# rvp-group/srrg2_proslam

Measured on AMD Instinct MI355X. Metric: tracked frames/sec on KITTI-00 stereo (1241x376, ~2k kp); SE(3) vs ref, higher is better.
Workload: dtype u64 popcount (Hamming) + f32 (projection, Jacobians, 6x6 normal equations)

## Files before the change

### srrg2_proslam_amd/csrc/align.hip

```cpp
#include "prs_device.h"
#include "prs_host.h"
#include "prs_se3.h"

#include <math.h>
#include <string.h>

#include <type_traits>
#include <vector>

namespace prs {

constexpr int kAlignThreads = 256;
constexpr int kTerms        = 29;
constexpr uint32_t kNoneU32 = 0xffffffffu;
constexpr float kFltMax     = 3.402823466e+38f;

typedef unsigned int au32x4 __attribute__((ext_vector_type(4)));

struct AlignShared {
  float X[16];
  float A[16];
  float Sinv[16];
  float T[16];
  float Tprev[16];
// ... 1495 lines not shown
      const float dn2 = ((((dx6[0] * dx6[0] + dx6[1] * dx6[1]) + dx6[2] * dx6[2]) + dx6[3] * dx6[3]) + dx6[4] * dx6[4]) + dx6[5] * dx6[5];
      const bool small_step = g.a.step_norm_exit > 0.0f && step_ok && dn2 < g.a.step_norm_exit * g.a.step_norm_exit;
      uint32_t changed_bits = 0;
#pragma unroll
      for (int i = 0; i < 16; ++i) {
        changed_bits |= __float_as_uint(X[i]) ^ __float_as_uint(sh.X[i]);
        sh.X[i] = X[i];
      }
      float a16[16];
      pose_to_camera(g.a, sh.Sinv, X, a16);
#pragma unroll
      for (int i = 0; i < 16; ++i) {
        sh.A[i] = a16[i];
      }
      sh.decision = ((g.a.stop_at_fixed_point && changed_bits == 0u && (sh.converged || inlier_run)) || (small_step && (sh.converged || inlier_run))) ? 1 : 0;
    }
    __syncthreads();
    ALIGN_ACC(acc_solve);
    if (sh.decision) {
      if (!inlier_run && inlier_run_length(g.a) > 0) {
        it_align = g.a.max_iterations - 1;
        continue;
      }
      ++it_align;
      break;
    }
  }

  __syncthreads();
  if (g.mode == PRS_MODE_ALIGN && !split_search && g.a.keep_only_inlier_correspondences && sh.have_cls && !sh.error) {
    const int nc = sh.n_corr;
    int base     = 0;
    for (int c0 = 0; c0 < nc; c0 += T) {
      const int c     = c0 + tid;
      const bool keep = c < nc && clsbuf[c] == 0;
      prs_corr cr;
      if (keep) {
        cr = gcorr[c];
      }
      const unsigned long long bal = __ballot(keep);
      if (lane == 0) {
        sh.wave_tot[wave] = __popcll(bal);
      }
      __syncthreads();
      int pos = base + __popcll(bal & ((1ull << lane) - 1ull));
      for (int w = 0; w < T / 64; ++w) {
        pos += w < wave ? sh.wave_tot[w] : 0;
        base += sh.wave_tot[w];
      }
      if (keep) {
        gcorr[pos] = cr;
      }
      __syncthreads();
    }
    if (tid == 0) {
      sh.n_corr = base;
    }
    __syncthreads();
  }

  __syncthreads();
  if (tid < 16) {
    if (!split_search) {
      g.b.X[(size_t) frame * 16 + tid] = sh.X[tid];
    }
    gstate->local_map_in_sensor[tid]          = sh.T[tid];
    gstate->local_map_in_sensor_previous[tid] = sh.Tprev[tid];
  }
  for (int i = tid; i < 36; i += T) {
    gres->H[i] = sh.H[i];
  }
  if (tid < 6) {
    gres->b[tid] = sh.b[tid];
  }
  if (tid == 0) {
    gstate->search_radius_pixels = sh.radius;
    gstate->current_iteration    = sh.it;
    gstate->descriptor_distance  = sh.dd;
    gstate->database_leaf_range  = sh.kd_range;
    gstate->has_converged        = sh.converged;
    gstate->config_changed       = sh.config_changed;
    gstate->num_recomputes       = sh.num_recomputes;
    gstate->reserved             = (gstate->reserved & ~1) | sh.no_prune;
    g.b.n_corr[frame]            = sh.n_corr;
    gres->chi_inliers            = sh.chi_in;
    gres->chi_total              = sh.chi_tot;
    gres->mean_disparity         = sh.mean_disp;
    gres->num_inliers            = sh.n_inl;
    gres->num_outliers           = sh.n_out;
    gres->num_invalid            = sh.n_inv;
    gres->num_correspondences    = sh.n_corr;
    gres->status                 = sh.n_inl >= g.a.min_num_inliers ? 1 : 0;
    gres->iterations             = g.mode == PRS_MODE_ALIGN ? (ran_inlier_phase ? max_it : g.a.max_iterations) : 1;
    gres->iterations_executed    = executed;
    gres->warnings               = sh.error ? sh.error : sh.flags;
    if (split_search) {
      ctl->flags |= sh.flags;
      ctl->need_search = 0;
      gres->warnings   = sh.error ? sh.error : ctl->flags;
    }
    if (g.stamps) {
      unsigned long long* st = g.stamps + (size_t) frame * 16;
      st[0] = 0;
      for (int i = 0; i < 9; ++i) {
        st[i + 1] = st[i] + sh.stamp_acc[i];
      }
    }
  }
}

constexpr int kGnThreads = 128;
constexpr int kGnSlots   = 8;

struct GnShared {
  float X[16], T[16], Tprev[16];
  float H[36], b[6];
  float chi_in, chi_tot;
  float fcnt[3];
  float pad0;
  float A[16];
  float Sinv[16];
  float wsum[32];
  unsigned long long it;
  int converged, need_search, n_inl, n_out, n_inv, stop, flags;
  int pose_ok;
  int wave_tot[4];
};
static_assert(offsetof(GnShared, b) == offsetof(GnShared, H) + 36 * sizeof(float) && offsetof(GnShared, chi_in) == offsetof(GnShared, b) + 6 * sizeof(float) &&
                offsetof(GnShared, chi_tot) == offsetof(GnShared, chi_in) + sizeof(float) && offsetof(GnShared, fcnt) == offsetof(GnShared, chi_tot) + sizeof(float),
              "the summed slots are written through GnShared::H");

__device__ __forceinline__ bool gn_advance(const prs_aligner_params& a, const int extra, int& it_align, bool fixed_point, const int n_inl) {
  const bool was_inlier_run = it_align >= a.max_iterations;
  ++it_align;
  if (fixed_point && !was_inlier_run && extra > 0) {
    it_align    = a.max_iterations;
    fixed_point = false;
  }
  if (fixed_point) {
    return true;
  }
  if (it_align == a.max_iterations && extra > 0) {
    return n_inl < a.min_num_inliers;
  }
  return it_align >= a.max_iterations + extra;
}

template <bool SHIPPED_FORMS = false, int PLAIN = 0>
__device__ __forceinline__ void gn_solve_wave(const AlignArgs& g, GnShared& sh, const int frame, const int nc, const int stid, const bool inlier_run) {
  const int lane = stid;
  if (sh.pose_ok) {
    const int rrow = lane < 6 ? lane : 5;
    const int blk  = rrow >= 3 ? 1 : 0;
    const int ci   = rrow - 3 * blk;
    const float* Yb = &sh.H[18 * blk];
    const float Ri0 = sh.A[ci], Ri1 = sh.A[4 + ci], Ri2 = sh.A[8 + ci];
    float o[6];
#pragma unroll
    for (int cb = 0; cb < 2; ++cb) {
      float v[3];
#pragma unroll
      for (int c = 0; c < 3; ++c) {
        v[c] = fmaf(Ri2, Yb[12 + 3 * cb + c], fmaf(Ri1, Yb[6 + 3 * cb + c], Ri0 * Yb[3 * cb + c]));
      }
#pragma unroll
      for (int j = 0; j < 3; ++j) {
        o[3 * cb + j] = fmaf(v[2], sh.A[8 + j], fmaf(v[1], sh.A[4 + j], v[0] * sh.A[j]));
      }
    }
    const float bb = fmaf(Ri2, sh.b[3 * blk + 2], fmaf(Ri1, sh.b[3 * blk + 1], Ri0 * sh.b[3 * blk]));
    __builtin_amdgcn_fence(__ATOMIC_RELEASE, "wavefront");
    __builtin_amdgcn_wave_barrier();
    __builtin_amdgcn_fence(__ATOMIC_ACQUIRE, "wavefront");
    if (lane < 6) {
      float2* hw = reinterpret_cast<float2*>(&sh.H[6 * rrow]);
      hw[0]      = make_float2(o[0], o[1]);
      hw[1]      = make_float2(o[2], o[3]);
      hw[2]      = make_float2(o[4], o[5]);
      sh.b[rrow] = bb;
    }
    __builtin_amdgcn_fence(__ATOMIC_RELEASE, "wavefront");
    __builtin_amdgcn_wave_barrier();
    __builtin_amdgcn_fence(__ATOMIC_ACQUIRE, "wavefront");
  }
  if (stid == 0) {
    const int cc = (int) sh.fcnt[0];
    sh.n_inl     = cc & ((int) kClsOutUnit - 1);
    sh.n_out     = cc / (int) kClsOutUnit;
    sh.n_inv     = nc - sh.n_inl - sh.n_out;
  }
  {
    const int prow  = lane < 3 ? lane : 2;
    const float4 xr = *reinterpret_cast<const float4*>(&sh.X[4 * prow]);
    float H[36], b[6];
#pragma unroll
    for (int i = 0; i < 36; ++i) {
      H[i] = sh.H[i];
    }
#pragma unroll
    for (int i = 0; i < 6; ++i) {
      b[i] = sh.b[i];
    }
    if (PLAIN == 0 && g.b.prior) {
      const float* pr = g.b.prior + (size_t) frame * 42;
#pragma unroll
      for (int i = 0; i < 36; ++i) {
        H[i] += pr[i];
      }
#pragma unroll
      for (int i = 0; i < 6; ++i) {
        b[i] += pr[36 + i];
      }
    }
    if (PLAIN == 2 || (PLAIN == 0 && g.a.enable_motion_prior)) {
      float X[16];
#pragma unroll
      for (int i = 0; i < 16; ++i) {
        X[i] = sh.X[i];
      }
      add_motion_prior(g.a, g.prior_mean ? g.prior_mean + (size_t) frame * 16 : nullptr, X, H, b);
    }
    auto bcast = [](const float v, const int l) -> float { return __int_as_float(__builtin_amdgcn_readlane(__float_as_int(v), l)); };
    float dx[6];
    const bool ok = ldlt_solve6(H, b, g.a.damping, dx, !SHIPPED_FORMS && g.a.damping_form == PRS_DAMPING_IDENTITY);
    bool small_step = false;
    if (g.a.step_norm_exit > 0.0f) {
      const float n2 = ((((dx[0] * dx[0] + dx[1] * dx[1]) + dx[2] * dx[2]) + dx[3] * dx[3]) + dx[4] * dx[4]) + dx[5] * dx[5];
      small_step     = ok && n2 < g.a.step_norm_exit * g.a.step_norm_exit;
    }
    float D[16];
    tnq2t(dx, D);
    float4 xn;
    xn.x = (xr.x * D[0] + xr.y * D[4]) + xr.z * D[8];
    xn.y = (xr.x * D[1] + xr.y * D[5]) + xr.z * D[9];
    xn.z = (xr.x * D[2] + xr.y * D[6]) + xr.z * D[10];
    xn.w = ((xr.x * D[3] + xr.y * D[7]) + xr.z * D[11]) + xr.w;
    xn.x = ok ? xn.x : xr.x;
    xn.y = ok ? xn.y : xr.y;
    xn.z = ok ? xn.z : xr.z;
    xn.w = ok ? xn.w : xr.w;
    const uint32_t changed = (__float_as_uint(xn.x) ^ __float_as_uint(xr.x)) | (__float_as_uint(xn.y) ^ __float_as_uint(xr.y)) |
                             (__float_as_uint(xn.z) ^ __float_as_uint(xr.z)) | (__float_as_uint(xn.w) ^ __float_as_uint(xr.w));
    const bool any_changed = (__ballot(changed != 0u) & 7ull) != 0ull;
    float4 an = xn;
    if (PLAIN == 0 && g.a.with_sensor) {
      const float4 sr = *reinterpret_cast<const float4*>(&sh.Sinv[4 * prow]);
      const float4 x0 = {bcast(xn.x, 0), bcast(xn.y, 0), bcast(xn.z, 0), bcast(xn.w, 0)};
      const float4 x1 = {bcast(xn.x, 1), bcast(xn.y, 1), bcast(xn.z, 1), bcast(xn.w, 1)};
      const float4 x2 = {bcast(xn.x, 2), bcast(xn.y, 2), bcast(xn.z, 2), bcast(xn.w, 2)};
      an.x = (sr.x * x0.x + sr.y * x1.x) + sr.z * x2.x;
      an.y = (sr.x * x0.y + sr.y * x1.y) + sr.z * x2.y;
      an.z = (sr.x * x0.z + sr.y * x1.z) + sr.z * x2.z;
      an.w = ((sr.x * x0.w + sr.y * x1.w) + sr.z * x2.w) + sr.w;
    }
    const float rs = (an.x + an.y) + (an.z + an.w);
    const float fs = (bcast(rs, 0) + bcast(rs, 1)) + bcast(rs, 2);
    if (lane < 3) {
      *reinterpret_cast<float4*>(&sh.X[4 * lane]) = xn;
      *reinterpret_cast<float4*>(&sh.A[4 * lane]) = an;
    }
    if (stid == 0) {
      sh.stop    = ((g.a.stop_at_fixed_point && !any_changed && (sh.converged || inlier_run)) || (small_step && (sh.converged || inlier_run))) ? 1 : 0;
      sh.pose_ok = (fs - fs) == 0.0f ? 1 : 0;
    }
  }
}

__device__ __forceinline__ void gn_finder_bookkeeping(const AlignArgs& g, GnShared& sh, const int stid, const int nc, const int it_align, const int extra,
                                                      const bool fixed_point) {
    int next        = it_align;
    const bool over = gn_advance(g.a, extra, next, fixed_point, sh.n_inl);
    if (!over && next < g.a.max_iterations) {
      if (stid < 16) {
        sh.T[stid] = sh.A[stid];
      }
      if (!sh.converged) {
        const unsigned long long k  = g.f.number_of_solver_iterations_per_projection;
        const unsigned long long it = sh.it;
        if (k == 0 || it % k == 0 || it == 1) {
          if (stid == 0) {
            sh.need_search = 1;
          }
        } else {
          if (stid < 16) {
            sh.Tprev[stid] = sh.A[stid];
          }
          if (stid == 0) {
            sh.it = it + 1;
            if (nc == 0) {
              sh.flags |= PRS_WARN_NO_MATCHES;
            }
          }
        }
      } else if (stid == 0 && nc == 0) {
        sh.flags |= PRS_WARN_NO_MATCHES;
      }
    }
}

constexpr int kGnLdsSlots = 4;
constexpr size_t gn_lds_bytes(const int lds_slots) {
  return ((sizeof(GnShared) + 15) / 16) * 16 + (size_t) (lds_slots * 128 + 64) * 2 * sizeof(float4);
}
template <int SLOTS, int DIM, bool KEEP_CLS, int LDS_SLOTS = kGnLdsSlots, int WAVES = 4, int PLAIN = 0>
__global__ __launch_bounds__(128, WAVES) void gn_kernel(const AlignArgs g) {
  constexpr int THREADS = 128;
  constexpr int kGnLdsSlots = LDS_SLOTS;
  constexpr int kGnLdsRows  = LDS_SLOTS * 128 + 64;
  extern __shared__ __attribute__((aligned(16))) unsigned char smem[];
  const int tid   = threadIdx.x;
  const int lane  = tid & 63;
  const int wave  = tid >> 6;
  const int frame = blockIdx.x;
  const int solver = frame & 1;
  const int stid   = tid - 64 * solver;
  FrameCtl* ctl    = g.ctl + frame;
  constexpr int LS_IDX = (SLOTS < LDS_SLOTS ? SLOTS : LDS_SLOTS) + 1;
  const size_t fbase                    = (size_t) frame * (size_t) g.b.fixed_stride;
  const prs_corr* __restrict__ gcorr_in = g.b.corr + fbase;
  int fi[LS_IDX], mi[LS_IDX];
#pragma unroll
  for (int k = 0; k < LS_IDX; ++k) {
    const int c  = k * 128 + tid;
    const int cc = c < g.b.fixed_stride ? c : 0;
    fi[k]        = gcorr_in[cc].fixed_idx;
    mi[k]        = gcorr_in[cc].moving_idx;
  }
  if (ctl->done || ctl->need_search) {
    return;
  }
  GnShared& sh             = *reinterpret_cast<GnShared*>(smem);
  prs_pcf_state* gstate    = g.b.state + frame;
  prs_align_result* gres   = g.b.result + frame;
  const float4* gops       = g.ops + (size_t) frame * (size_t) g.max_fixed * 2;
  const int nc             = g.b.n_corr[frame];
  const float mean_dsp     = gres->mean_disparity;

  if (tid < 16) {
    sh.X[tid]     = g.b.X[(size_t) frame * 16 + tid];
    sh.T[tid]     = gstate->local_map_in_sensor[tid];
    sh.Tprev[tid] = gstate->local_map_in_sensor_previous[tid];
  }
  if (tid == 0) {
    sh.it          = gstate->current_iteration;
    sh.converged   = gstate->has_converged;
    sh.need_search = 0;
    sh.flags       = 0;
    sh.n_inl       = ctl->n_inl;
    sh.n_out       = ctl->n_out;
    sh.n_inv       = ctl->n_inv;
    sh.chi_in      = gres->chi_inliers;
    sh.chi_tot     = gres->chi_total;
    sh.stop        = 0;
    const float* gx = g.b.X + (size_t) frame * 16;
    float x[16], a16[16], si[16];
#pragma unroll
    for (int i = 0; i < 16; ++i) {
      x[i] = gx[i];
    }
    se3_inverse(g.a.sensor_in_robot, si);
    pose_to_camera(g.a, si, x, a16);
#pragma unroll
    for (int i = 0; i < 16; ++i) {
      sh.Sinv[i] = si[i];
      sh.A[i]    = a16[i];
    }
    const PoseRegs x0 = {a16[0], a16[1], a16[2], a16[3], a16[4], a16[5], a16[6], a16[7], a16[8], a16[9], a16[10], a16[11]};
    sh.pose_ok        = pose_is_finite(x0) ? 1 : 0;
  }
  for (int i = tid; i < 36; i += THREADS) {
    sh.H[i] = gres->H[i];
  }
  if (tid < 6) {
    sh.b[tid] = gres->b[tid];
  }
  constexpr int LS = SLOTS < kGnLdsSlots ? SLOTS : kGnLdsSlots;
  float4* lz = reinterpret_cast<float4*>(smem + ((sizeof(GnShared) + 15) / 16) * 16);
  constexpr int LROWS = SLOTS <= kGnLdsSlots ? SLOTS * THREADS : kGnLdsRows;
  float4* lp = lz + LROWS;
  const float4* __restrict__ gfix = reinterpret_cast<const float4*>(g.b.fixed) + fbase;
  const float4* __restrict__ gmov = reinterpret_cast<const float4*>(g.b.moving) + (size_t) frame * (size_t) g.b.moving_stride;
  if (nc > 0) {
    static_assert(LS_IDX == LS + 1, "index pairs of the parked rows");
    float4 zr[LS + 1], pr[LS + 1];
#pragma unroll
    for (int k = 0; k < LS + 1; ++k) {
      const bool live = k * THREADS + tid < nc;
      zr[k]           = gfix[live ? fi[k] : 0];
      pr[k]           = gmov[live ? mi[k] : 0];
    }
#pragma unroll
    for (int k = 0; k < LS + 1; ++k) {
      const int c = k * THREADS + tid;
      if (k * THREADS < nc && c < LROWS) {
        float4 z = c < nc ? zr[k] : make_float4(0.f, 0.f, 0.f, 0.f);
        z.w      = parked_translation_weight(g.a, z, mean_dsp, DIM != 0 ? 0 : g.a.translation_weight_form);
        lz[c]    = z;
        lp[c]    = c < nc ? pr[k] : make_float4(0.f, 0.f, 1.f, 1.f);
      }
    }
  }
  if (SLOTS > kGnLdsSlots) {
    float4* wops = g.ops + (size_t) frame * (size_t) g.max_fixed * 2;
#pragma unroll
    for (int k = LS; k < SLOTS; ++k) {
      const int c = k * THREADS + tid;
      if (c >= LROWS && c < nc) {
        const int fi    = gcorr_in[c].fixed_idx, mi = gcorr_in[c].moving_idx;
        float4 z        = gfix[fi];
        z.w             = parked_translation_weight(g.a, z, mean_dsp, DIM != 0 ? 0 : g.a.translation_weight_form);
        wops[2 * c]     = z;
        wops[2 * c + 1] = gmov[mi];
      }
    }
  }
  const int my_slot = (lane >> 1) & 31;
  const int sum_dst = gn_slot_destination(my_slot, (lane & 1) != 0);
  __syncthreads();

  int it_align = ctl->it_align;
  int executed = ctl->executed;
  bool done    = false;
  const int extra = PLAIN != 0 ? 0 : inlier_run_length(g.a);
  uint32_t cls_bits = 0;
  bool have_cls     = false;


  while (true) {
    ++executed;
    if (nc < g.a.min_num_correspondences) {
      if (tid == 0) {
        sh.n_inl = sh.n_out = sh.n_inv = 0;
        sh.chi_in = sh.chi_tot = 0.0f;
        sh.stop = (g.a.stop_at_fixed_point && (sh.converged || it_align >= g.a.max_iterations)) ? 1 : 0;
      }
      for (int i = tid; i < 36; i += THREADS) {
        sh.H[i] = 0.0f;
      }
      if (tid < 6) {
        sh.b[tid] = 0.0f;
      }
      have_cls = false;
      __syncthreads();
      if (wave == solver) {
        gn_finder_bookkeeping(g, sh, stid, nc, it_align, extra, sh.stop != 0);
      }
      __syncthreads();
    } else {
      const bool inlier_run = PLAIN == 0 && it_align >= g.a.max_iterations;
      have_cls              = true;
      cls_bits              = 0;
      const PoseRegs pose = {sh.A[0], sh.A[1], sh.A[2], sh.A[3], sh.A[4], sh.A[5], sh.A[6], sh.A[7], sh.A[8], sh.A[9], sh.A[10], sh.A[11]};
      const bool pose_ok  = __builtin_amdgcn_readfirstlane(sh.pose_ok) != 0;
      f2 acc[kPairs];
#pragma unroll
      for (int i = 0; i < kPairs; ++i) {
        acc[i] = f2{0.0f, 0.0f};
      }
      float code = 0.0f;
      if (pose_ok) {
#pragma unroll
        for (int k = 0; k < SLOTS; ++k) {
          const int c0 = k * THREADS;
          if (k == 0 || c0 + 64 * wave < nc) {
            const int c = c0 + tid;
            float4 z, p;
            if (k < LS || (k == LS && c0 + 64 * wave < LROWS)) {
              z = lz[c];
              p = lp[c];
            } else {
              const int cs = cold_copy(c);
              z   = c < nc ? gops[2 * cs] : make_float4(0.f, 0.f, 0.f, 1.f);
              p   = c < nc ? gops[2 * cs + 1] : make_float4(0.f, 0.f, 1.f, 1.f);
            }
            int cls;
            factor_accumulate<DIM, true>(g.a, pose, z, p, mean_dsp, c < nc, acc, code, cls, inlier_run);
            if (KEEP_CLS) {
              cls_bits |= (uint32_t) (cls & 3) << (2 * k);
            }
          }
        }
      } else if (KEEP_CLS) {
#pragma unroll
        for (int k = 0; k < SLOTS; ++k) {
          if (k * THREADS + tid < nc) {
            cls_bits |= 2u << (2 * k);
          }
        }
      }
      acc[kSlotCls >> 1].x = code;
      float tot = wave_sum_slots(acc, lane);
      if (wave != solver) {
        sh.wsum[my_slot] = tot;
      }
      __syncthreads();
      if (wave == solver) {
        tot = tot + sh.wsum[my_slot];
        tot = tot + 0.0f;
        (&sh.H[0])[sum_dst] = tot;
        __builtin_amdgcn_fence(__ATOMIC_RELEASE, "wavefront");
        __builtin_amdgcn_wave_barrier();
        __builtin_amdgcn_fence(__ATOMIC_ACQUIRE, "wavefront");
        gn_solve_wave<DIM != 0, PLAIN>(g, sh, frame, nc, stid, inlier_run);
        __builtin_amdgcn_fence(__ATOMIC_RELEASE, "wavefront");
        __builtin_amdgcn_wave_barrier();
        __builtin_amdgcn_fence(__ATOMIC_ACQUIRE, "wavefront");
        gn_finder_bookkeeping(g, sh, stid, nc, it_align, extra, sh.stop != 0);
      }
      __syncthreads();
    }
    if (gn_advance(g.a, extra, it_align, sh.stop != 0, sh.n_inl)) {
      done = true;
      break;
    }
    if (it_align < g.a.max_iterations && sh.need_search) {
      break;
    }
  }

  int nc_out = nc;
  __syncthreads();
  if (KEEP_CLS && done && g.a.keep_only_inlier_correspondences && have_cls) {
    prs_corr* __restrict__ gcorr = g.b.corr + (size_t) frame * (size_t) g.b.fixed_stride;
    int base                     = 0;
#pragma unroll
    for (int k = 0; k < SLOTS; ++k) {
      const int c0 = k * THREADS;
      if (c0 < nc) {
        const int c     = c0 + tid;
        const bool keep = c < nc && ((cls_bits >> (2 * k)) & 3u) == 0u;
        prs_corr cr;
        if (keep) {
          cr = gcorr[c];
        }
        const unsigned long long bal = __ballot(keep);
        if (lane == 0) {
          sh.wave_tot[wave] = __popcll(bal);
        }
        __syncthreads();
        int pos = base + __popcll(bal & ((1ull << lane) - 1ull));
#pragma unroll
        for (int w = 0; w < THREADS / 64; ++w) {
          pos += w < wave ? sh.wave_tot[w] : 0;
          base += sh.wave_tot[w];
        }
        if (keep) {
          gcorr[pos] = cr;
        }
        __syncthreads();
      }
    }
    nc_out = base;
  }

  __syncthreads();
  if (tid < 16) {
    g.b.X[(size_t) frame * 16 + tid]           = sh.X[tid];
    gstate->local_map_in_sensor[tid]          = sh.T[tid];
    gstate->local_map_in_sensor_previous[tid] = sh.Tprev[tid];
  }
  for (int i = tid; i < 36; i += THREADS) {
    const int r = i / 6, c = i - 6 * r;
    gres->H[i]  = sh.H[r >= c ? i : 6 * c + r];
  }
  if (tid < 6) {
    gres->b[tid] = sh.b[tid];
  }
  if (tid == 0) {
    gstate->current_iteration = sh.it;
    gres->chi_inliers         = sh.chi_in;
    gres->chi_total           = sh.chi_tot;
    gres->num_inliers         = sh.n_inl;
    gres->num_outliers        = sh.n_out;
    gres->num_invalid         = sh.n_inv;
    gres->num_correspondences = nc_out;
    if (nc_out != nc) {
      g.b.n_corr[frame] = nc_out;
    }
    gres->status              = sh.n_inl >= g.a.min_num_inliers ? 1 : 0;
    gres->iterations          = it_align > g.a.max_iterations ? g.a.max_iterations + extra : g.a.max_iterations;
    gres->iterations_executed = executed;
    ctl->flags |= sh.flags;
    gres->warnings   = ctl->flags;
    ctl->it_align    = it_align;
    ctl->executed    = executed;
    ctl->n_inl       = sh.n_inl;
    ctl->n_out       = sh.n_out;
    ctl->n_inv       = sh.n_inv;
    ctl->need_search = done ? 0 : 1;
    ctl->done        = done ? 1 : 0;
    if (!done) {
      atomicAdd(g.pending, 1);
    }
  }
}

__global__ void split_init_kernel(FrameCtl* ctl, prs_align_result* res, int* pending, int batch) {
  const int i = blockIdx.x * blockDim.x + threadIdx.x;
  if (i < batch) {
    FrameCtl c;
    c.it_align    = 0;
    c.need_search = 1;
    c.done        = 0;
    c.executed    = 0;
    c.flags       = 0;
    c.n_inl = c.n_out = c.n_inv = 0;
    c.db_ready                  = 0;
    ctl[i]                      = c;
    prs_align_result r;
    for (int k = 0; k < 36; ++k) {
      r.H[k] = 0.0f;
    }
    for (int k = 0; k < 6; ++k) {
      r.b[k] = 0.0f;
    }
    r.chi_inliers = r.chi_total = r.mean_disparity = 0.0f;
    r.num_inliers = r.num_outliers = r.num_invalid = r.num_correspondences = 0;
    r.status = r.iterations = r.iterations_executed = r.warnings = 0;
    res[i]                                                        = r;
  }
  if (i == 0) {
    *pending = 0;
  }
}

__global__ void gn_step_kernel(const float* H, const float* b, float damping, int identity_damping, float* X, int* ok) {
  float h[36], bb[6], x[16];
  for (int i = 0; i < 36; ++i) {
    h[i] = H[i];
  }
  for (int i = 0; i < 6; ++i) {
    bb[i] = b[i];
  }
  for (int i = 0; i < 16; ++i) {
    x[i] = X[i];
  }
  const bool r = gn_step(h, bb, damping, x, identity_damping != 0);
  for (int i = 0; i < 16; ++i) {
    X[i] = x[i];
  }
  *ok = r ? 1 : 0;
}

static inline uint32_t align_up16(uint32_t v) {
  return (v + 15u) / 16u * 16u;
}

struct SplitJob {
  bool active = false;
  void* own[3]        = {nullptr, nullptr, nullptr};
  size_t own_bytes[3] = {0, 0, 0};
  hipStream_t stream  = nullptr;
  hipStream_t capture_stream = nullptr;
  ~SplitJob() {
    for (void* p : own) {
      if (p) {
        (void) hipFree(p);
      }
    }
  }
  void* buffer(hipStream_t s, int i, size_t bytes) {
    if (bytes <= own_bytes[i]) {
      return own[i];
    }
    if (own[i]) {
      (void) hipStreamSynchronize(s);
      (void) hipFree(own[i]);
      own[i]       = nullptr;
      own_bytes[i] = 0;
    }
    const size_t want = bytes + bytes / 4 + 4096;
    if (hipMalloc(&own[i], want) != hipSuccess) {
      own[i] = nullptr;
      return nullptr;
    }
    own_bytes[i] = want;
    return own[i];
  }
  AlignArgs g, gs;
  void (*search)(AlignArgs) = nullptr;
  void (*gn)(AlignArgs)     = nullptr;
  size_t lds_search = 0, lds_gn = 0;
  int total = 0, limit = 0;
  int enqueued = 0;
  int ev_used = 0;
  int rounds_timed = 0;
  bool stamps = false;
};
static int split_rounds(prs_context* ctx, SplitJob* job, int rounds);

int align_batch_launch(prs_context* ctx, const prs_pcf_params* finder, const prs_aligner_params* aligner, const prs_align_batch* batch, int mode, int rounds) {
  if (ctx->align_job && static_cast<SplitJob*>(ctx->align_job)->active) {
    return ctx_fail(ctx, PRS_ERR_UNSUPPORTED, "prs_align_batch_*: the previous batch of this context has not been finished (prs_align_batch_finish)");
  }
  if (!finder || !aligner || !batch || !batch->fixed || !batch->fixed_desc || !batch->n_fixed || !batch->moving ||
      !batch->moving_desc || !batch->n_moving || !batch->state || !batch->X || !batch->corr || !batch->n_corr || !batch->result) {
    return ctx_fail(ctx, PRS_ERR_NULL, "prs_align_batch_run: fixed, moving, correspondences, state or result not set");
  }
  if (mode < PRS_MODE_ALIGN || mode > PRS_MODE_LINEARIZE) {
    return ctx_fail(ctx, PRS_ERR_UNSUPPORTED, "prs_align_batch_run: unknown mode");
  }
  if (batch->batch <= 0) {
    return PRS_OK;
  }
  if (batch->fixed_stride <= 0 || batch->fixed_stride > 32767 || batch->moving_stride <= 0 || batch->moving_stride > 65535) {
    return ctx_fail(ctx, PRS_ERR_UNSUPPORTED, "prs_align_batch_run: fixed_stride must be in [1,32767], moving_stride in [1,65535]");
  }
  if (finder->projector.canvas_rows <= 0 || finder->projector.canvas_rows > 8192 || finder->projector.canvas_cols <= 0 ||
      finder->projector.canvas_cols > 32767) {
    return ctx_fail(ctx, PRS_ERR_UNSUPPORTED, "prs_align_batch_run: projector canvas must be within 32767 x 8192");
  }
  if (finder->maximum_search_radius_pixels > 16383 || finder->search_type < PRS_SEARCH_KDTREE || finder->search_type > PRS_SEARCH_RHOMBUS) {
    return ctx_fail(ctx, PRS_ERR_UNSUPPORTED, "prs_align_batch_run: search radius > 16383 px or unknown search type");
  }
  if (aligner->factor_type != PRS_FACTOR_MONO && aligner->factor_type != PRS_FACTOR_DEPTH && aligner->factor_type != PRS_FACTOR_STEREO) {
    return ctx_fail(ctx, PRS_ERR_UNSUPPORTED, "prs_align_batch_run: factor_type must be 2, 3 or 4");
  }
  if ((aligner->kernel_weight_form != PRS_KERNEL_WEIGHT_INV_CHI && aligner->kernel_weight_form != PRS_KERNEL_WEIGHT_TAU_OVER_CHI) ||
      (aligner->damping_form != PRS_DAMPING_DIAG && aligner->damping_form != PRS_DAMPING_IDENTITY) ||
      (aligner->translation_weight_form != PRS_TRANSLATION_WEIGHT_OFFSET && aligner->translation_weight_form != PRS_TRANSLATION_WEIGHT_CLAMP)) {
    return ctx_fail(ctx, PRS_ERR_UNSUPPORTED, "prs_align_batch_run: unknown kernel_weight_form / damping_form / translation_weight_form");
  }
  AlignArgs g;
  g.f          = *finder;
  g.a          = *aligner;
  g.b          = *batch;
  g.mode       = mode;
  g.no_prefilter = ctx->no_prefilter ? 1 : 0;
  g.narrow_prefilter_limit = ctx->prefilter_96_limit;
  g.prior_mean = batch->prior_mean;
  g.rows_table = finder->projector.canvas_rows;
  const int max_fixed = batch->max_fixed > 0 && batch->max_fixed < batch->fixed_stride ? batch->max_fixed : batch->fixed_stride;
  g.max_fixed       = max_fixed;
  const uint32_t nf = (uint32_t) max_fixed;
  const uint32_t R  = (uint32_t) g.rows_table;
  uint32_t lut_cap  = 2u * (uint32_t) finder->maximum_search_radius_pixels + 1u;
  if (lut_cap > 2048u) {
    lut_cap = 2048u;
  }
  g.lut_cap = (int) lut_cap;
  int sy = 4, sx = 4;
  auto cells_of = [&](int shift_y, int shift_x, int& ncy, int& ncx) {
    ncy = ((int) R + (1 << shift_y) - 1) >> shift_y;
    ncx = (finder->projector.canvas_cols + (1 << shift_x) - 1) >> shift_x;
    return ncy * ncx;
  };
  int ncy = 0, ncx = 0;
  while (cells_of(sy, sx, ncy, ncx) > 2048) {
    if (ncy > ncx) {
      ++sy;
    } else {
      ++sx;
    }
  }
  g.cell_sy  = sy;
  g.cell_sx  = sx;
  g.cell_ncy = ncy;
  g.cell_ncx = ncx;
  g.ncells   = ncy * ncx;
  const bool kdtree         = finder->search_type == PRS_SEARCH_KDTREE;
  const uint32_t cs_entries = kdtree && nf + 4u > (uint32_t) g.ncells + 2u ? nf + 4u : (uint32_t) g.ncells + 2u;
  auto carve = [&](AlignArgs& g, bool with_operands) -> size_t {
    uint32_t off = 0;
    g.off_db       = off; off = align_up16(off + (nf + 1) * 8);
    g.off_inv      = off; off = align_up16(off + nf * 2);
    g.off_cellstart = off; off = align_up16(off + cs_entries * 2);
    g.off_cfix     = off; off = align_up16(off + (with_operands ? nf * 16 : 0));
    g.off_cmov     = off; off = align_up16(off + (with_operands ? nf * 16 : 0));
    g.off_cls      = off; off = align_up16(off + (with_operands ? nf : 0));
    g.off_sh       = off; off = align_up16(off + (uint32_t) sizeof(AlignShared));
    g.off_u        = off;
    uint32_t u = off;
    g.off_fdesc  = u; u = align_up16(u + nf * 32);
    g.off_fuv    = u; u = align_up16(u + (finder->search_type == PRS_SEARCH_KDTREE ? nf * 8 : 0));
    g.off_best   = u; u = align_up16(u + nf * 4);
    g.off_second = u; u = align_up16(u + nf * 4);
    g.off_lut    = u; u = align_up16(u + lut_cap * 2);
    g.off_surv   = u; u = align_up16(u + (uint32_t) (with_operands ? kAlignThreads : kSearchThreads) * (uint32_t) g.surv_slots * 2);
    g.off_terms = off;
    uint32_t terms_bytes       = kTerms * kAlignThreads * 4;
    const uint32_t histcap     = (R > (uint32_t) g.ncells ? R : (uint32_t) g.ncells) + 2;
    const uint32_t build_bytes = histcap * 4 + (nf + 2) * 2 * 3 + (R + 2) * 2 + 16;
    if (build_bytes > terms_bytes) {
      terms_bytes = build_bytes;
    }
    if (nf * 4 + 160 > terms_bytes) {
      terms_bytes = nf * 4 + 160;
    }
    const uint32_t kd_bytes = (uint32_t) kd_open_capacity((int) nf) * (40 + 7 * 4) + (nf + 2) * 2 * 3 + 64;
    if (kdtree && kd_bytes > terms_bytes) {
      terms_bytes = kd_bytes;
    }
    const uint32_t t_end = align_up16(off + terms_bytes);
    return u > t_end ? u : t_end;
  };
  g.surv_slots     = 4;
  const size_t lds = carve(g, true);
  if (lds > 160 * 1024) {
    return ctx_fail(ctx, PRS_ERR_UNSUPPORTED, "prs_align_batch_run: fixed cloud does not fit the 160 KiB LDS (lower max_fixed)");
  }
  g.stamps = ctx_stamps(ctx, (size_t) batch->batch * 16 * sizeof(unsigned long long));
  g.ops     = nullptr;
  g.ctl     = nullptr;
  g.pending = nullptr;
  g.dbcache = nullptr;
  g.db_blob = 0;
  hipStream_t stream = ctx_stream(ctx);
  hipError_t e;
  if (max_fixed >= (int) kClsOutUnit) {
    return ctx_fail(ctx, PRS_ERR_UNSUPPORTED, "prs_align_batch_run: max_fixed must be below 2048");
  }
  const bool stamps_split = g.stamps && ctx->stamps_split;
  const bool split = mode == PRS_MODE_ALIGN && !ctx_fused_align(ctx) && max_fixed <= kGnThreads * kGnSlots && (!g.stamps || stamps_split);
  if (!split) {
    auto kernel = align_kernel<kAlignThreads, false, -1>;
    e           = hipFuncSetAttribute(reinterpret_cast<const void*>(kernel), hipFuncAttributeMaxDynamicSharedMemorySize, (int) lds);
    if (e != hipSuccess) {
      return ctx_fail_hip(ctx, e, "prs_align_batch_run attribute");
    }
    hipLaunchKernelGGL(kernel, dim3(batch->batch), dim3(kAlignThreads), lds, stream, g);
    e = hipGetLastError();
    if (e != hipSuccess) {
      return ctx_fail_hip(ctx, e, "prs_align_batch_run launch");
    }
    if (g.stamps) {
      ctx_report_stamps(ctx, batch->batch, 10, "align (fused, 256 threads): finder | linearize + in-wave reduction | cross-wave sum | GN solve || of finder: lattice build | projection+search | staging (keys, fixed rows -> LDS) | filter | commit");
    }
    return PRS_OK;
  }
  SplitJob* job = static_cast<SplitJob*>(ctx->align_job);
  if (!job) {
    job                 = new SplitJob();
    ctx->align_job      = job;
    ctx->align_job_free = [](void* p) { delete static_cast<SplitJob*>(p); };
  }
  const size_t ops_bytes = (size_t) batch->batch * (size_t) max_fixed * 2 * sizeof(float4);
  const size_t ctl_bytes = (size_t) batch->batch * sizeof(FrameCtl) + 256;
  unsigned char* small   = static_cast<unsigned char*>(job->buffer(stream, 0, ctl_bytes));
  g.ops                  = static_cast<float4*>(job->buffer(stream, 1, ops_bytes));
  if (!small || !g.ops) {
    return ctx_fail(ctx, PRS_ERR_HIP, "prs_align_batch_run: split-pipeline scratch allocation failed");
  }
  g.pending = reinterpret_cast<int*>(small);
  g.ctl     = reinterpret_cast<FrameCtl*>(small + 256);
  AlignArgs gs = g;
  gs.mode      = kModeSplitSearch;
  gs.surv_slots = 8;
  size_t lds_search = carve(gs, false);
  gs.surv_slots     = 4;
  {
    const size_t lds4 = carve(gs, false);
    if ((160u * 1024u) / lds_search == (160u * 1024u) / lds4 && finder->search_type != PRS_SEARCH_KDTREE) {
      gs.surv_slots = 8;
      lds_search    = carve(gs, false);
    } else {
      lds_search = lds4;
    }
  }
  gs.db_blob = align_up16(gs.off_cellstart + cs_entries * 2) - gs.off_db;
  gs.dbcache = static_cast<unsigned char*>(job->buffer(stream, 2, (size_t) batch->batch * gs.db_blob));
  if (!gs.dbcache) {
    return ctx_fail(ctx, PRS_ERR_HIP, "prs_align_batch_run: lattice cache allocation failed");
  }
  const bool wide_slots = gs.surv_slots == 8;
  auto skernel = finder->search_type == PRS_SEARCH_CIRCLE
                   ? (wide_slots ? align_kernel<kSearchThreads, true, PRS_SEARCH_CIRCLE, 8> : align_kernel<kSearchThreads, true, PRS_SEARCH_CIRCLE, 4>)
                   : (finder->search_type == PRS_SEARCH_SQUARE
                        ? (wide_slots ? align_kernel<kSearchThreads, true, PRS_SEARCH_SQUARE, 8> : align_kernel<kSearchThreads, true, PRS_SEARCH_SQUARE, 4>)
                        : (finder->search_type == PRS_SEARCH_RHOMBUS
                             ? (wide_slots ? align_kernel<kSearchThreads, true, PRS_SEARCH_RHOMBUS, 8> : align_kernel<kSearchThreads, true, PRS_SEARCH_RHOMBUS, 4>)
                             : align_kernel<kSearchThreads, true, PRS_SEARCH_KDTREE, 4>));
  e = hipFuncSetAttribute(reinterpret_cast<const void*>(skernel), hipFuncAttributeMaxDynamicSharedMemorySize, (int) lds_search);
  if (e != hipSuccess) {
    return ctx_fail_hip(ctx, e, "prs_align_batch_run attribute");
  }
  hipLaunchKernelGGL(split_init_kernel, dim3((batch->batch + 255) / 256), dim3(256), 0, stream, g.ctl, batch->result, g.pending, batch->batch);
  const bool fast = aligner->factor_type == PRS_FACTOR_STEREO && !aligner->keep_only_inlier_correspondences && aligner->kernel_weight_form == PRS_KERNEL_WEIGHT_INV_CHI &&
                    aligner->damping_form == PRS_DAMPING_DIAG && aligner->translation_weight_form == PRS_TRANSLATION_WEIGHT_OFFSET;
  int n_cu = 0;
  (void) hipDeviceGetAttribute(&n_cu, hipDeviceAttributeMultiprocessorCount, ctx->device);
  const bool lone = fast && batch->batch <= 2 * (n_cu > 0 ? n_cu : 256) && !ctx->no_lone_gn;
  const bool five = fast && !lone && max_fixed > 4 * 128;
  const bool lean  = !batch->prior && !aligner->with_sensor && !aligner->enable_inlier_only_runs;
  const bool plain = lean && !aligner->enable_motion_prior;
  const bool mprior = lean && aligner->enable_motion_prior;
  const bool depth = aligner->factor_type == PRS_FACTOR_DEPTH && aligner->kernel_weight_form == PRS_KERNEL_WEIGHT_INV_CHI && aligner->damping_form == PRS_DAMPING_DIAG;
  auto gnk        = lone ? (max_fixed <= 4 * 128 ? (plain ? gn_kernel<4, PRS_FACTOR_STEREO, false, kGnLdsSlots, 1, 1> : gn_kernel<4, PRS_FACTOR_STEREO, false, kGnLdsSlots, 1>)
                                                 : (plain ? gn_kernel<8, PRS_FACTOR_STEREO, false, kGnLdsSlots, 1, 1> : gn_kernel<8, PRS_FACTOR_STEREO, false, kGnLdsSlots, 1>))
                         : (max_fixed <= 4 * 128 ? (fast ? (plain ? gn_kernel<4, PRS_FACTOR_STEREO, false, kGnLdsSlots, 4, 1> : (mprior ? gn_kernel<4, PRS_FACTOR_STEREO, false, kGnLdsSlots, 4, 2> : gn_kernel<4, PRS_FACTOR_STEREO, false>))
                                                         : (depth ? gn_kernel<4, PRS_FACTOR_DEPTH, true> : gn_kernel<4, 0, true>))
                                                 : (fast ? (plain ? gn_kernel<8, PRS_FACTOR_STEREO, false, 3, 5, 1> : (mprior ? gn_kernel<8, PRS_FACTOR_STEREO, false, 3, 5, 2> : gn_kernel<8, PRS_FACTOR_STEREO, false, 3, 5>))
                                                         : (depth ? gn_kernel<8, PRS_FACTOR_DEPTH, true> : gn_kernel<8, 0, true>)));
  const size_t lds_gn = gn_lds_bytes(five ? 3 : kGnLdsSlots);
  job->active      = true;
  job->stream      = stream;
  job->capture_stream = stream;
  job->g           = g;
  job->gs          = gs;
  job->search      = reinterpret_cast<void (*)(AlignArgs)>(skernel);
  job->gn          = reinterpret_cast<void (*)(AlignArgs)>(gnk);
  job->lds_search  = lds_search;
  job->lds_gn      = lds_gn;
  job->total       = 0;
  job->limit       = 2 * (aligner->max_iterations + inlier_run_length(*aligner)) + 8;
  job->ev_used     = 0;
  job->rounds_timed = 0;
  job->stamps      = stamps_split;
  job->enqueued    = rounds > 0 ? rounds : 5;
  return split_rounds(ctx, job, job->enqueued);
}

static int split_rounds(prs_context* ctx, SplitJob* job, int rounds) {
  hipStream_t stream = job->stream;
  auto tick = [&]() {
    if (ctx->timing && job->ev_used < 3 * 64) {
      if (!ctx->timing_ev[job->ev_used]) {
        (void) hipEventCreate(&ctx->timing_ev[job->ev_used]);
      }
      (void) hipEventRecord(ctx->timing_ev[job->ev_used], stream);
      ++job->ev_used;
    }
  };
  const int batch = job->g.b.batch;
  for (int r = 0; r < rounds; ++r) {
    (void) hipMemsetAsync(job->g.pending, 0, sizeof(int), stream);
    tick();
    hipLaunchKernelGGL(job->search, dim3(batch), dim3(kSearchThreads), job->lds_search, stream, job->gs);
    tick();
    if (job->stamps) {
      ctx_report_stamps(ctx, batch, 10, "search launch (split): - | - | - | - || lattice build | projection+search | staging (keys, fixed rows -> LDS) | filter | commit");
    }
    hipLaunchKernelGGL(job->gn, dim3(batch), dim3(kGnThreads), job->lds_gn, stream, job->g);
    tick();
    ++job->total;
  }
  const hipError_t e = hipGetLastError();
  if (e != hipSuccess) {
    job->active = false;
    return ctx_fail_hip(ctx, e, "prs_align_batch_run split launch");
  }
  return PRS_OK;
}

int align_batch_finish(prs_context* ctx) {
  SplitJob* job = static_cast<SplitJob*>(ctx->align_job);
  if (!job || !job->active) {
    return PRS_OK;
  }
  hipStream_t stream = job->stream;
  auto collect = [&]() {
    for (int i = 0; i + 2 < job->ev_used; i += 3) {
      float a = 0.f, b = 0.f;
      if (hipEventElapsedTime(&a, ctx->timing_ev[i], ctx->timing_ev[i + 1]) == hipSuccess &&
          hipEventElapsedTime(&b, ctx->timing_ev[i + 1], ctx->timing_ev[i + 2]) == hipSuccess) {
        ctx->t_search_ms += a;
        ctx->t_gn_ms += b;
        ++ctx->n_search;
        ++ctx->n_gn;
        const int round = job->rounds_timed < 15 ? job->rounds_timed : 15;
        ctx->t_search_round[round] += a;
        ctx->t_gn_round[round] += b;
      }
      ++job->rounds_timed;
    }
    job->ev_used = 0;
  };
  for (;;) {
    int pending  = 0;
    hipError_t e = hipMemcpyAsync(&pending, job->g.pending, sizeof(int), hipMemcpyDeviceToHost, stream);
    if (e == hipSuccess) {
      e = hipStreamSynchronize(stream);
    }
    if (e != hipSuccess) {
      job->active = false;
      return ctx_fail_hip(ctx, e, "prs_align_batch_finish: completion check");
    }
    collect();
    if (pending == 0) {
      break;
    }
    if (job->total > job->limit) {
      job->active = false;
      return ctx_fail(ctx, PRS_ERR_HIP, "prs_align_batch_finish: split pipeline did not finish");
    }
    const int rc = split_rounds(ctx, job, 4);
    if (rc != PRS_OK) {
      return rc;
    }
  }
  job->active = false;
  if (ctx->timing) {
    ++ctx->n_batches_timed;
  }
  return PRS_OK;
}

int align_batch_rearm(prs_context* ctx, hipStream_t replay_stream) {
  SplitJob* job = static_cast<SplitJob*>(ctx->align_job);
  if (!job || !job->gn) {
    return ctx_fail(ctx, PRS_ERR_UNSUPPORTED, "prs_align_batch_rearm: no batch has been enqueued on this context");
  }
  if (job->active) {
    return ctx_fail(ctx, PRS_ERR_UNSUPPORTED, "prs_align_batch_rearm: the previous batch has not been finished");
  }
  job->stream       = replay_stream ? replay_stream : job->capture_stream;
  job->active       = true;
  job->total        = job->enqueued;
  job->ev_used      = 0;
  job->rounds_timed = 0;
  return PRS_OK;
}

bool align_job_active(const prs_context* ctx) {
  const SplitJob* job = static_cast<const SplitJob*>(ctx->align_job);
  return job && job->active;
}

__global__ __launch_bounds__(256) void recip_selftest_kernel(unsigned long long* counts) {
  const uint32_t stride = gridDim.x * blockDim.x;
  unsigned long long differ = 0, fast = 0;
  for (uint64_t i = (uint64_t) blockIdx.x * blockDim.x + threadIdx.x; i < (1ull << 32); i += stride) {
    const float x  = __uint_as_float((uint32_t) i);
    const float ax = __builtin_fabsf(x);
    const bool short_form = __ballot(!(ax >= 0x1p-126f && ax < 0x1p126f)) == 0ull;
    const uint32_t got = __float_as_uint(recip_exact(x)), want = __float_as_uint(1.0f / x);
    const bool both_nan = (got & 0x7fffffffu) > 0x7f800000u && (want & 0x7fffffffu) > 0x7f800000u;
    differ += (got != want && !both_nan) ? 1ull : 0ull;
    fast += short_form ? 1ull : 0ull;
  }
  if (differ) {
    atomicAdd(&counts[0], differ);
  }
  atomicAdd(&counts[1], fast);
}

int recip_selftest_launch(prs_context* ctx, unsigned long long* d_counts) {
  hipLaunchKernelGGL(recip_selftest_kernel, dim3(256 * 32), dim3(256), 0, ctx_stream(ctx), d_counts);
  hipError_t e = hipGetLastError();
  if (e != hipSuccess) {
    return ctx_fail_hip(ctx, e, "prs_selftest_reciprocal launch");
  }
  return PRS_OK;
}

int gn_step_launch(prs_context* ctx, const float* dH, const float* db, float damping, int damping_form, float* dX, int* dok) {
  hipLaunchKernelGGL(gn_step_kernel, dim3(1), dim3(1), 0, ctx_stream(ctx), dH, db, damping, damping_form == PRS_DAMPING_IDENTITY ? 1 : 0, dX, dok);
  hipError_t e = hipGetLastError();
  if (e != hipSuccess) {
    return ctx_fail_hip(ctx, e, "prs_gn_step launch");
  }
  return PRS_OK;
}

}
```

Before: 1.771 million.

## Run plain stereo Gauss-Newton frame on a single wave instead of two

Adds a one-wave (64-thread) path for the plain fast stereo GN kernel. Each lane handles two halves of the correspondence slots sequentially, parking some rows in LDS, some in registers and the rest in global memory. Block-wide barriers and the cross-wave partial-sum exchange are replaced by wave-local fences. The aim is to remove inter-wave synchronisation and the idle solver wave, at the cost of doubling per-lane linearisation work and adding register pressure. Optional cycle-stamp instrumentation is also added behind a compile flag.

After: 1.801 million (median of 6 runs). 1.7% higher.

```diff
diff --git a/srrg2_proslam_amd/csrc/align.hip b/srrg2_proslam_amd/csrc/align.hip
--- a/srrg2_proslam_amd/csrc/align.hip
+++ b/srrg2_proslam_amd/csrc/align.hip
@@ -1821,8 +1821,304 @@
 constexpr size_t gn_lds_bytes(const int lds_slots) {
   return ((sizeof(GnShared) + 15) / 16) * 16 + (size_t) (lds_slots * 128 + 64) * 2 * sizeof(float4);
 }
+
+#ifndef PRS_GN_STAMPS
+#define PRS_GN_STAMPS 0
+#endif
+enum { kGnStLin = 0, kGnStReduce, kGnStExchange, kGnStSolve, kGnStBook, kGnStPhases, kGnStSlot0 = 10 };
+#if PRS_GN_STAMPS
+__device__ __forceinline__ unsigned long long gn_stamp_now() {
+  unsigned long long t;
+  __builtin_amdgcn_sched_barrier(0);
+  asm volatile("s_memtime %0\n\ts_waitcnt lgkmcnt(0)" : "=s"(t)::"memory");
+  __builtin_amdgcn_sched_barrier(0);
+  return t;
+}
+#define GN_ST_DECL() unsigned long long gn_st_[kGnStPhases] = {0, 0, 0, 0, 0}, gn_st_prev_ = 0, gn_st_its_ = 0
+#define GN_ST_MARK() (gn_st_prev_ = gn_stamp_now())
+#define GN_ST_ACC(v) do { const unsigned long long now_ = gn_stamp_now(); gn_st_[v] += now_ - gn_st_prev_; gn_st_prev_ = now_; } while (0)
+#define GN_ST_ITER() (++gn_st_its_)
+#define GN_ST_STORE(first_lane) do { if (g.stamps && (first_lane)) { unsigned long long* st_ = g.stamps + (size_t) frame * 16 + kGnStSlot0; \
+  for (int i_ = 0; i_ < kGnStPhases; ++i_) { st_[i_] += gn_st_[i_]; } st_[kGnStPhases] += gn_st_its_; } } while (0)
+#else
+#define GN_ST_DECL() do { } while (0)
+#define GN_ST_MARK() do { } while (0)
+#define GN_ST_ACC(v) do { } while (0)
+#define GN_ST_ITER() do { } while (0)
+#define GN_ST_STORE(first_lane) do { } while (0)
+#endif
+
+constexpr int kGnWaveLdsSlots = 4;
+constexpr int kGnWaveRegSlots = 4;
+#ifndef PRS_GN_TWO_WAVES
+#define PRS_GN_TWO_WAVES 0
+#endif
+constexpr bool gn_one_wave(const int slots, const int dim, const bool keep_cls, const int lds_slots, const int waves, const int plain) {
+  return !PRS_GN_TWO_WAVES && slots == 8 && dim == PRS_FACTOR_STEREO && !keep_cls && lds_slots == 3 && waves == 5 && plain == 1;
+}
+constexpr size_t gn_wave_lds_bytes() {
+  return ((sizeof(GnShared) + 15) / 16) * 16 + (size_t) (kGnWaveLdsSlots * 64) * 2 * sizeof(float4);
+}
+__device__ __forceinline__ void wave_lds_sync() {
+  __builtin_amdgcn_fence(__ATOMIC_RELEASE, "wavefront");
+  __builtin_amdgcn_wave_barrier();
+  __builtin_amdgcn_fence(__ATOMIC_ACQUIRE, "wavefront");
+}
+template <int SLOTS, int DIM>
+__device__ __forceinline__ void gn_frame_wave(const AlignArgs& g) {
+  constexpr int PLAIN = 1;
+  constexpr int NV    = 2 * SLOTS;
+  constexpr int LV    = kGnWaveLdsSlots;
+  constexpr int PV    = kGnWaveLdsSlots + kGnWaveRegSlots;
+  static_assert(PV <= NV && LV % 2 == 0 && PV % 2 == 0, "parked wave slots: whole slots of the two-wave form");
+  extern __shared__ __attribute__((aligned(16))) unsigned char smem[];
+  const int lane  = threadIdx.x;
+  const int frame = blockIdx.x;
+  FrameCtl* ctl   = g.ctl + frame;
+  const size_t fbase                    = (size_t) frame * (size_t) g.b.fixed_stride;
+  const prs_corr* __restrict__ gcorr_in = g.b.corr + fbase;
+  int fi[PV], mi[PV];
+#pragma unroll
+  for (int v = 0; v < PV; ++v) {
+    const int c  = v * 64 + lane;
+    const int cc = c < g.b.fixed_stride ? c : 0;
+    fi[v]        = gcorr_in[cc].fixed_idx;
+    mi[v]        = gcorr_in[cc].moving_idx;
+  }
+  if (ctl->done || ctl->need_search) {
+    return;
+  }
+  GnShared& sh           = *reinterpret_cast<GnShared*>(smem);
+  prs_pcf_state* gstate  = g.b.state + frame;
+  prs_align_result* gres = g.b.result + frame;
+  const float4* gops     = g.ops + (size_t) frame * (size_t) g.max_fixed * 2;
+  const int nc           = g.b.n_corr[frame];
+  const float mean_dsp   = gres->mean_disparity;
+
+  if (lane < 16) {
+    sh.X[lane]     = g.b.X[(size_t) frame * 16 + lane];
+    sh.T[lane]     = gstate->local_map_in_sensor[lane];
+    sh.Tprev[lane] = gstate->local_map_in_sensor_previous[lane];
+  }
+  if (lane == 0) {
+    sh.it          = gstate->current_iteration;
+    sh.converged   = gstate->has_converged;
+    sh.need_search = 0;
+    sh.flags       = 0;
+    sh.n_inl       = ctl->n_inl;
+    sh.n_out       = ctl->n_out;
+    sh.n_inv       = ctl->n_inv;
+    sh.chi_in      = gres->chi_inliers;
+    sh.chi_tot     = gres->chi_total;
+    sh.stop        = 0;
+    const float* gx = g.b.X + (size_t) frame * 16;
+    float x[16], a16[16], si[16];
+#pragma unroll
+    for (int i = 0; i < 16; ++i) {
+      x[i] = gx[i];
+    }
+    se3_inverse(g.a.sensor_in_robot, si);
+    pose_to_camera(g.a, si, x, a16);
+#pragma unroll
+    for (int i = 0; i < 16; ++i) {
+      sh.Sinv[i] = si[i];
+      sh.A[i]    = a16[i];
+    }
+    const PoseRegs x0 = {a16[0], a16[1], a16[2], a16[3], a16[4], a16[5], a16[6], a16[7], a16[8], a16[9], a16[10], a16[11]};
+    sh.pose_ok        = pose_is_finite(x0) ? 1 : 0;
+  }
+  if (lane < 36) {
+    sh.H[lane] = gres->H[lane];
+  }
+  if (lane < 6) {
+    sh.b[lane] = gres->b[lane];
+  }
+  float4* lz = reinterpret_cast<float4*>(smem + ((sizeof(GnShared) + 15) / 16) * 16);
+  float4* lp = lz + LV * 64;
+  float4 rz[kGnWaveRegSlots], rp[kGnWaveRegSlots];
+#pragma unroll
+  for (int j = 0; j < kGnWaveRegSlots; ++j) {
+    rz[j] = make_float4(0.f, 0.f, 0.f, 1.f);
+    rp[j] = make_float4(0.f, 0.f, 1.f, 1.f);
+  }
+  const float4* __restrict__ gfix = reinterpret_cast<const float4*>(g.b.fixed) + fbase;
+  const float4* __restrict__ gmov = reinterpret_cast<const float4*>(g.b.moving) + (size_t) frame * (size_t) g.b.moving_stride;
+  {
+    float4 zr[PV], pr[PV];
+#pragma unroll
+    for (int v = 0; v < PV; ++v) {
+      const bool live = v * 64 + lane < nc;
+      zr[v]           = gfix[live ? fi[v] : 0];
+      pr[v]           = gmov[live ? mi[v] : 0];
+    }
+#pragma unroll
+    for (int v = 0; v < PV; ++v) {
+      const int c = v * 64 + lane;
+      if (v < 2 || v * 64 < nc) {
+        float4 z = c < nc ? zr[v] : make_float4(0.f, 0.f, 0.f, 0.f);
+        z.w      = parked_translation_weight(g.a, z, mean_dsp, 0);
+        const float4 p = c < nc ? pr[v] : make_float4(0.f, 0.f, 1.f, 1.f);
+        if (v < LV) {
+          lz[c] = z;
+          lp[c] = p;
+        } else {
+          rz[v - LV] = z;
+          rp[v - LV] = p;
+        }
+      }
+    }
+  }
+  {
+    float4* wops = g.ops + (size_t) frame * (size_t) g.max_fixed * 2;
+#pragma unroll
+    for (int v = PV; v < NV; ++v) {
+      const int c = v * 64 + lane;
+      if (c < nc) {
+        const int f = gcorr_in[c].fixed_idx, m = gcorr_in[c].moving_idx;
+        float4 z        = gfix[f];
+        z.w             = parked_translation_weight(g.a, z, mean_dsp, 0);
+        wops[2 * c]     = z;
+        wops[2 * c + 1] = gmov[m];
+      }
+    }
+  }
+  const int sum_dst = gn_slot_destination((lane >> 1) & 31, (lane & 1) != 0);
+  __syncthreads();
+
+  int it_align    = ctl->it_align;
+  int executed    = ctl->executed;
+  bool done       = false;
+  constexpr int extra = 0;
+  GN_ST_DECL();
+
+  while (true) {
+    ++executed;
+    if (nc < g.a.min_num_correspondences) {
+      if (lane == 0) {
+        sh.n_inl = sh.n_out = sh.n_inv = 0;
+        sh.chi_in = sh.chi_tot = 0.0f;
+        sh.stop = (g.a.stop_at_fixed_point && (sh.converged || it_align >= g.a.max_iterations)) ? 1 : 0;
+      }
+      if (lane < 36) {
+        sh.H[lane] = 0.0f;
+      }
+      if (lane < 6) {
+        sh.b[lane] = 0.0f;
+      }
+      wave_lds_sync();
+      gn_finder_bookkeeping(g, sh, lane, nc, it_align, extra, sh.stop != 0);
+      wave_lds_sync();
+    } else {
+      GN_ST_MARK();
+      const PoseRegs pose = {sh.A[0], sh.A[1], sh.A[2], sh.A[3], sh.A[4], sh.A[5], sh.A[6], sh.A[7], sh.A[8], sh.A[9], sh.A[10], sh.A[11]};
+      const bool pose_ok = __builtin_amdgcn_readfirstlane(sh.pose_ok) != 0;
+      float tot = 0.0f;
+      if (pose_ok) {
+#pragma unroll 1
+        for (int h = 0; h < 2; ++h) {
+          f2 acc[kPairs];
+#pragma unroll
+          for (int i = 0; i < kPairs; ++i) {
+            acc[i] = f2{0.0f, 0.0f};
+          }
+          float code = 0.0f;
+#pragma unroll
+          for (int k = 0; k < SLOTS; ++k) {
+            const int v = 2 * k + h;
+            if (k == 0 || v * 64 < nc) {
+              const int c = v * 64 + lane;
+              float4 z, p;
+              if (2 * k < LV) {
+                z = lz[c];
+                p = lp[c];
+              } else if (2 * k < PV) {
+                const int j = 2 * k - LV;
+                z = h ? rz[j + 1] : rz[j];
+                p = h ? rp[j + 1] : rp[j];
+              } else {
+                const int cs = cold_copy(c);
+                z = c < nc ? gops[2 * cs] : make_float4(0.f, 0.f, 0.f, 1.f);
+                p = c < nc ? gops[2 * cs + 1] : make_float4(0.f, 0.f, 1.f, 1.f);
+              }
+              int cls;
+              factor_accumulate<DIM, true>(g.a, pose, z, p, mean_dsp, c < nc, acc, code, cls, false);
+            }
+          }
+          acc[kSlotCls >> 1].x = code;
+          GN_ST_ACC(kGnStLin);
+          const float t = wave_sum_slots(acc, lane);
+          tot           = h == 0 ? t : tot + t;
+          GN_ST_ACC(kGnStReduce);
+        }
+      }
+      tot                 = tot + 0.0f;
+      (&sh.H[0])[sum_dst] = tot;
+      wave_lds_sync();
+      GN_ST_ACC(kGnStExchange);
+      gn_solve_wave<DIM != 0, PLAIN>(g, sh, frame, nc, lane, false);
+      wave_lds_sync();
+      GN_ST_ACC(kGnStSolve);
+      gn_finder_bookkeeping(g, sh, lane, nc, it_align, extra, sh.stop != 0);
+      wave_lds_sync();
+      GN_ST_ACC(kGnStBook);
+      GN_ST_ITER();
+    }
+    if (gn_advance(g.a, extra, it_align, sh.stop != 0, sh.n_inl)) {
+      done = true;
+      break;
+    }
+    if (it_align < g.a.max_iterations && sh.need_search) {
+      break;
+    }
+  }
+  GN_ST_STORE(lane == 0);
+
+  __syncthreads();
+  if (lane < 16) {
+    g.b.X[(size_t) frame * 16 + lane]          = sh.X[lane];
+    gstate->local_map_in_sensor[lane]          = sh.T[lane];
+    gstate->local_map_in_sensor_previous[lane] = sh.Tprev[lane];
+  }
+  if (lane < 36) {
+    const int r = lane / 6, c = lane - 6 * r;
+    gres->H[lane] = sh.H[r >= c ? lane : 6 * c + r];
+  }
+  if (lane < 6) {
+    gres->b[lane] = sh.b[lane];
+  }
+  if (lane == 0) {
+    gstate->current_iteration = sh.it;
+    gres->chi_inliers         = sh.chi_in;
+    gres->chi_total           = sh.chi_tot;
+    gres->num_inliers         = sh.n_inl;
+    gres->num_outliers        = sh.n_out;
+    gres->num_invalid         = sh.n_inv;
+    gres->num_correspondences = nc;
+    gres->status              = sh.n_inl >= g.a.min_num_inliers ? 1 : 0;
+    gres->iterations          = it_align > g.a.max_iterations ? g.a.max_iterations + extra : g.a.max_iterations;
+    gres->iterations_executed = executed;
+    ctl->flags |= sh.flags;
+    gres->warnings   = ctl->flags;
+    ctl->it_align    = it_align;
+    ctl->executed    = executed;
+    ctl->n_inl       = sh.n_inl;
+    ctl->n_out       = sh.n_out;
+    ctl->n_inv       = sh.n_inv;
+    ctl->need_search = done ? 0 : 1;
+    ctl->done        = done ? 1 : 0;
+    if (!done) {
+      atomicAdd(g.pending, 1);
+    }
+  }
+}
+
 template <int SLOTS, int DIM, bool KEEP_CLS, int LDS_SLOTS = kGnLdsSlots, int WAVES = 4, int PLAIN = 0>
-__global__ __launch_bounds__(128, WAVES) void gn_kernel(const AlignArgs g) {
+__global__ __launch_bounds__(gn_one_wave(SLOTS, DIM, KEEP_CLS, LDS_SLOTS, WAVES, PLAIN) ? 64 : 128,
+                             gn_one_wave(SLOTS, DIM, KEEP_CLS, LDS_SLOTS, WAVES, PLAIN) ? 4 : WAVES) void gn_kernel(const AlignArgs g) {
+  if constexpr (gn_one_wave(SLOTS, DIM, KEEP_CLS, LDS_SLOTS, WAVES, PLAIN)) {
+    gn_frame_wave<SLOTS, DIM>(g);
+    return;
+  } else {
   constexpr int THREADS = 128;
   constexpr int kGnLdsSlots = LDS_SLOTS;
   constexpr int kGnLdsRows  = LDS_SLOTS * 128 + 64;
@@ -1943,6 +2239,7 @@
   const int extra = PLAIN != 0 ? 0 : inlier_run_length(g.a);
   uint32_t cls_bits = 0;
   bool have_cls     = false;
+  GN_ST_DECL();
 
 
   while (true) {
@@ -1971,6 +2268,7 @@
       cls_bits              = 0;
       const PoseRegs pose = {sh.A[0], sh.A[1], sh.A[2], sh.A[3], sh.A[4], sh.A[5], sh.A[6], sh.A[7], sh.A[8], sh.A[9], sh.A[10], sh.A[11]};
       const bool pose_ok  = __builtin_amdgcn_readfirstlane(sh.pose_ok) != 0;
+      GN_ST_MARK();
       f2 acc[kPairs];
 #pragma unroll
       for (int i = 0; i < kPairs; ++i) {
@@ -2008,7 +2306,9 @@
         }
       }
       acc[kSlotCls >> 1].x = code;
+      GN_ST_ACC(kGnStLin);
       float tot = wave_sum_slots(acc, lane);
+      GN_ST_ACC(kGnStReduce);
       if (wave != solver) {
         sh.wsum[my_slot] = tot;
       }
@@ -2020,13 +2320,17 @@
         __builtin_amdgcn_fence(__ATOMIC_RELEASE, "wavefront");
         __builtin_amdgcn_wave_barrier();
         __builtin_amdgcn_fence(__ATOMIC_ACQUIRE, "wavefront");
+        GN_ST_ACC(kGnStExchange);
         gn_solve_wave<DIM != 0, PLAIN>(g, sh, frame, nc, stid, inlier_run);
         __builtin_amdgcn_fence(__ATOMIC_RELEASE, "wavefront");
         __builtin_amdgcn_wave_barrier();
         __builtin_amdgcn_fence(__ATOMIC_ACQUIRE, "wavefront");
+        GN_ST_ACC(kGnStSolve);
         gn_finder_bookkeeping(g, sh, stid, nc, it_align, extra, sh.stop != 0);
       }
       __syncthreads();
+      GN_ST_ACC(kGnStBook);
+      GN_ST_ITER();
     }
     if (gn_advance(g.a, extra, it_align, sh.stop != 0, sh.n_inl)) {
       done = true;
@@ -2037,6 +2341,7 @@
     }
   }
 
+  GN_ST_STORE(stid == 0);
   int nc_out = nc;
   __syncthreads();
   if (KEEP_CLS && done && g.a.keep_only_inlier_correspondences && have_cls) {
@@ -2112,6 +2417,7 @@
       atomicAdd(g.pending, 1);
     }
   }
+  }
 }
 
 __global__ void split_init_kernel(FrameCtl* ctl, prs_align_result* res, int* pending, int batch) {
@@ -2200,6 +2506,7 @@
   void (*search)(AlignArgs) = nullptr;
   void (*gn)(AlignArgs)     = nullptr;
   size_t lds_search = 0, lds_gn = 0;
+  int gn_threads = kGnThreads;
   int total = 0, limit = 0;
   int enqueued = 0;
   int ev_used = 0;
@@ -2393,6 +2700,11 @@
   if (e != hipSuccess) {
     return ctx_fail_hip(ctx, e, "prs_align_batch_run attribute");
   }
+#if PRS_GN_STAMPS
+  if (stamps_split) {
+    (void) hipMemsetAsync(g.stamps, 0, (size_t) batch->batch * 16 * sizeof(unsigned long long), stream);
+  }
+#endif
   hipLaunchKernelGGL(split_init_kernel, dim3((batch->batch + 255) / 256), dim3(256), 0, stream, g.ctl, batch->result, g.pending, batch->batch);
   const bool fast = aligner->factor_type == PRS_FACTOR_STEREO && !aligner->keep_only_inlier_correspondences && aligner->kernel_weight_form == PRS_KERNEL_WEIGHT_INV_CHI &&
                     aligner->damping_form == PRS_DAMPING_DIAG && aligner->translation_weight_form == PRS_TRANSLATION_WEIGHT_OFFSET;
@@ -2410,7 +2722,8 @@
                                                          : (depth ? gn_kernel<4, PRS_FACTOR_DEPTH, true> : gn_kernel<4, 0, true>))
                                                  : (fast ? (plain ? gn_kernel<8, PRS_FACTOR_STEREO, false, 3, 5, 1> : (mprior ? gn_kernel<8, PRS_FACTOR_STEREO, false, 3, 5, 2> : gn_kernel<8, PRS_FACTOR_STEREO, false, 3, 5>))
                                                          : (depth ? gn_kernel<8, PRS_FACTOR_DEPTH, true> : gn_kernel<8, 0, true>)));
-  const size_t lds_gn = gn_lds_bytes(five ? 3 : kGnLdsSlots);
+  const bool one_wave = !lone && five && plain && gn_one_wave(8, PRS_FACTOR_STEREO, false, 3, 5, 1);
+  const size_t lds_gn = one_wave ? gn_wave_lds_bytes() : gn_lds_bytes(five ? 3 : kGnLdsSlots);
   job->active      = true;
   job->stream      = stream;
   job->capture_stream = stream;
@@ -2420,6 +2733,7 @@
   job->gn          = reinterpret_cast<void (*)(AlignArgs)>(gnk);
   job->lds_search  = lds_search;
   job->lds_gn      = lds_gn;
+  job->gn_threads  = one_wave ? 64 : kGnThreads;
   job->total       = 0;
   job->limit       = 2 * (aligner->max_iterations + inlier_run_length(*aligner)) + 8;
   job->ev_used     = 0;
@@ -2449,7 +2763,7 @@
     if (job->stamps) {
       ctx_report_stamps(ctx, batch, 10, "search launch (split): - | - | - | - || lattice build | projection+search | staging (keys, fixed rows -> LDS) | filter | commit");
     }
-    hipLaunchKernelGGL(job->gn, dim3(batch), dim3(kGnThreads), job->lds_gn, stream, job->g);
+    hipLaunchKernelGGL(job->gn, dim3(batch), dim3(job->gn_threads), job->lds_gn, stream, job->g);
     tick();
     ++job->total;
   }
@@ -2511,6 +2825,23 @@
   if (ctx->timing) {
     ++ctx->n_batches_timed;
   }
+#if PRS_GN_STAMPS
+  if (job->stamps) {
+    const int nb = job->g.b.batch;
+    std::vector<unsigned long long> h((size_t) nb * 16);
+    (void) hipMemcpy(h.data(), job->g.stamps, h.size() * sizeof(unsigned long long), hipMemcpyDeviceToHost);
+    double ph[kGnStPhases + 1] = {0, 0, 0, 0, 0, 0};
+    for (int b = 0; b < nb; ++b) {
+      for (int i = 0; i <= kGnStPhases; ++i) {
+        ph[i] += (double) h[(size_t) b * 16 + kGnStSlot0 + i];
+      }
+    }
+    const double its = ph[kGnStPhases] > 0 ? ph[kGnStPhases] : 1.0;
+    fprintf(stderr, "[prs gn stamps] %d threads/frame, %.0f linearising iterations; cycles per iteration: linearise %.0f | in-wave reduction %.0f | "
+                    "exchange + barrier %.0f | solve %.0f | bookkeeping %.0f\n",
+            job->gn_threads, its, ph[0] / its, ph[1] / its, ph[2] / its, ph[3] / its, ph[4] / its);
+  }
+#endif
   return PRS_OK;
 }
 
```
